# david-knigge/enf-pde

Measured on AMD Instinct MI355X. Metric: query-points/sec (ENF fit+decode) at 64 latents x 64^2 grid, higher is better.
Workload: dtype bf16; 1 GPU; navier_stokes_64x64_z64_b16_per_gpu; decoded_states=1, latents=64, signals_per_gpu=16, inner_steps=3, sampled_points=512, num_hidden=128, num_heads=2, latent_dim=16, num_out=1, invariant=rel_pos_periodic, hparams=config_navier_stokes.yaml:23-96 with 64 latents, parallelism=dp1 (signals sharded, no data-path collective in fit/decode)

## Files before the change

enf-pde_amd/_lib.py:

```python
import ctypes
import os

_HERE = os.path.dirname(os.path.abspath(__file__))
LIB_PATH = os.environ.get("ENF_HIP_LIB") or os.path.join(_HERE, "libenf_hip.so")
TEST_LIB_PATH = os.environ.get("ENF_HIP_TEST_LIB") or os.path.join(_HERE, "libenf_hip_test.so")

ENF_NUM_TENSORS = 46
PREC = {"f32": 0, "fp32": 0, "float32": 0, "bf16": 1, "bfloat16": 1}
INVARIANT_IDS = {"rel_pos_periodic": 0, "latitude_periodic": 1, "polar_periodic": 2, "ponita": 3,
                 "abs_pos": 4, "rel_pos": 5, "norm_rel_pos": 6, "ball": 7, "ball_lat": 8, "ponita_full": 9}

EXPORTS = ["enf_abi_version", "enf_strerror", "enf_invariant_dim", "enf_invariant_pose_dim", "enf_check_desc",
           "enf_packed_weight_bytes", "enf_pack_weights", "enf_workspace_bytes", "enf_forward",
           "enf_backward_latents", "enf_backward_latents_ex", "enf_forward_stages", "enf_lt_layout", "enf_lt_layout_ext", "enf_pack_pair", "enf_pair_forward",
           "enf_pair_backward", "enf_pair_backward_ex", "enf_pair_scratch_bytes", "enf_pair_variant", "enf_pair_partition", "enf_shared_forward_parts", "enf_shared_backward_applies", "enf_backward_weights", "enf_backward_weights_scratch_bytes",
           "enf_backward_all", "enf_backward_all_scratch_bytes", "enf_fit_step", "enf_fit_inputs",
           "enf_mse_value_grad",
           "enf_workspace_bytes_ex", "enf_fit_step_ex", "enf_mse_value_grad_ex", "enf_mse_scratch_bytes", "enf_pair_backward_ex2",
           "enf_pair_backward_scratch_bytes", "enf_backward_all_scratch_bytes_ex", "enf_backward_weights_ex",
           "enf_backward_weights_scratch_bytes_ex",
           "enf_fit_step_w", "enf_mse_value_grad_w", "enf_fit_inputs_w", "enf_fit_inputs_b",
           "enf_fit_step_cw", "enf_mse_value_grad_cw", "enf_fit_inputs_cw",
           "enf_fit_step_e", "enf_eval_loss", "enf_signal_sum",
           "enf_field_grad_workspace_bytes", "enf_field_grad", "enf_query_vjp",
# ... 160 lines not shown
    lib.enf_pair_forward.argtypes = [dp, vp, i64, vp, vp, vp, vp, vp, sz, vp]
    lib.enf_pair_backward.argtypes = [dp, vp, i64, vp, vp, vp, vp, vp, vp, ctypes.POINTER(vp), vp]
    lib.enf_pair_backward_ex.argtypes = [dp, vp, i64, vp, vp, vp, vp, vp, vp, ctypes.POINTER(vp), vp, vp]
    cu = ctypes.c_uint
    lib.enf_workspace_bytes_ex.restype = sz
    lib.enf_workspace_bytes_ex.argtypes = [dp, cu]
    lib.enf_fit_step_ex.argtypes = [dp, vp, i64, vp, vp, vp, vp, vp, ctypes.c_float, vp, vp, vp, vp, vp, sz, cu, vp]
    lib.enf_mse_scratch_bytes.restype = sz
    lib.enf_mse_scratch_bytes.argtypes = [sz, cu]
    lib.enf_mse_value_grad_ex.argtypes = [vp, vp, sz, ctypes.c_float, vp, vp, vp, sz, cu, vp]
    lib.enf_fit_step_w.argtypes = [dp, vp, i64, vp, vp, vp, vp, vp, ctypes.c_float, vp, vp, vp, vp, vp, sz, vp, cu, vp]
    lib.enf_mse_value_grad_w.argtypes = [vp, vp, vp, sz, ctypes.c_int32, ctypes.c_float, vp, vp, vp, sz, cu, vp]
    lib.enf_fit_inputs_w.argtypes = [ctypes.c_int, ctypes.POINTER(EnfFitComponent)] + [ctypes.c_int32] * 7 + [vp] * 9
    lib.enf_fit_inputs_b.argtypes = [ctypes.c_int, ctypes.POINTER(EnfFitComponent)] + [ctypes.c_int32] * 7 + [vp] * 9
    lib.enf_fit_step_cw.argtypes = [dp, vp, i64, vp, vp, vp, vp, vp, ctypes.c_float, vp, vp, vp, vp, vp, sz, vp, cu, vp]
    lib.enf_mse_value_grad_cw.argtypes = [vp, vp, vp, sz, ctypes.c_float, vp, vp, vp, sz, cu, vp]
    lib.enf_fit_inputs_cw.argtypes = [ctypes.c_int, ctypes.POINTER(EnfFitComponent)] + [ctypes.c_int32] * 7 + [vp] * 8 + [ctypes.c_int32, vp]
    lib.enf_fit_step_e.argtypes = [dp, vp, i64, vp, vp, vp, vp, vp, ctypes.c_float, vp, vp, vp, vp, vp, sz, vp, vp, vp, vp, cu, vp]
    lib.enf_eval_loss.argtypes = [dp, vp, i64] + [vp] * 11 + [sz, cu, vp]
    lib.enf_signal_sum.argtypes = [vp, ctypes.c_int32, ctypes.c_int32, ctypes.c_float, vp, vp]
    lib.enf_field_grad_workspace_bytes.restype = sz
    lib.enf_field_grad_workspace_bytes.argtypes = [dp, cu]
    lib.enf_field_grad.argtypes = [dp, vp, i64] + [vp] * 7 + [sz, cu, vp]
    lib.enf_query_vjp.argtypes = [dp, vp, i64] + [vp] * 8 + [sz, cu, vp]
    lib.enf_pair_backward_scratch_bytes.restype = sz
    lib.enf_pair_backward_scratch_bytes.argtypes = [dp, cu]
    lib.enf_pair_backward_ex2.argtypes = [dp, vp, i64, vp, vp, vp, vp, vp, vp, ctypes.POINTER(vp), vp, vp, sz, cu, vp]
    lib.enf_backward_all_scratch_bytes_ex.restype = sz
    lib.enf_backward_all_scratch_bytes_ex.argtypes = [dp, ci, cu]
    lib.enf_backward_weights_scratch_bytes_ex.restype = sz
    lib.enf_backward_weights_scratch_bytes_ex.argtypes = [dp, ci, cu]
    lib.enf_backward_weights_ex.argtypes = [dp, vp, i64, vp, vp, vp, vp, vp, vp, ctypes.POINTER(vp), vp, vp, sz, cu, vp]
    if test_hooks:
        for name in ("enf_debug_gemm", "enf_debug_pack", "enf_test_read_wave_sums"):
            getattr(lib, name).restype = ci
        lib.enf_debug_gemm.argtypes = [vp, vp, vp, ci, ci, ci, vp]
        lib.enf_debug_pack.argtypes = [vp, vp, ci, ci, ci, vp]
        lib.enf_test_read_wave_sums.argtypes = [vp]
    if lib.enf_abi_version() != 2:
        raise EnfError(f"{path}: ABI version mismatch")
    return lib


def check(rc):
    if rc == 0:
        return
    msg = load().enf_strerror(rc).decode()
    if rc == -2:
        raise ValueError(msg)
    if rc == -6:
        raise AssertionError(msg)
    if rc == -3:
        raise NotImplementedError(msg)
    raise EnfError(f"libenf_hip error {rc}: {msg}")


def launch(dev, fn, *args):
    import torch
    idx = dev.index if dev.index is not None else torch.cuda.current_device()
    if idx == torch.cuda.current_device():
        return check(fn(*args))
    with torch.cuda.device(idx):
        return check(fn(*args))


def ptr(t):
    return ctypes.c_void_p(t.data_ptr()) if t is not None else ctypes.c_void_p(0)

# ... 19 lines not shown
```

enf-pde_amd/csrc/enf_device.h:

```cpp
#pragma once
#include <hip/hip_runtime.h>
#include <type_traits>

#define DEV __device__ __forceinline__

typedef float f32x4 __attribute__((ext_vector_type(4)));
typedef __bf16 bf16x8 __attribute__((ext_vector_type(8)));
typedef __bf16 bf16x4 __attribute__((ext_vector_type(4)));
typedef unsigned int u32x4 __attribute__((ext_vector_type(4)));

constexpr int NWAVES = 8;
constexpr int NTHREADS = 64 * NWAVES;

template <bool BF16, int KB>
struct Frags {
  using T = typename std::conditional<BF16, bf16x8, f32x4>::type;
  T f[BF16 ? KB : 2 * KB];
};

typedef float f32x2_cvt __attribute__((ext_vector_type(2)));
typedef __bf16 bf16x2_cvt __attribute__((ext_vector_type(2)));
DEV unsigned bf16_pack2(float a, float b) {
  return __builtin_bit_cast(unsigned, __builtin_convertvector(f32x2_cvt{a, b}, bf16x2_cvt));
}
// ... 325 lines not shown
      const unsigned a = (unsigned)(uintptr_t)(lds_ptr_t)(const_cast<char*>(slot) + (lane << 4));
      f32x4 af[C::MTS];
      if constexpr (INIT == INIT_ZERO) {
        G::run_flip_zero(af, F.f, a);
      } else {
#pragma unroll
        for (int mt = 0; mt < C::MTS; ++mt) af[mt] = flip_init(sp * C::MTS + mt);
        G::run_flip(af, F.f, a);
      }
#pragma unroll
      for (int mt = 0; mt < C::MTS; ++mt) flip(sp * C::MTS + mt, af[mt]);
    } else {
      if constexpr (TRANS) gemm_stage<BF16, KBIN, C::MTS, INIT>(&acc[sp * C::MTS], F, slot, lane, bias + 16 * sp * C::MTS);
#pragma unroll
      for (int mt = 0; mt < C::MTS; ++mt) {
        f32x4 af = flip_init(sp * C::MTS + mt);
        gemm_tile_flip<BF16, KBIN>(af, F, slot, mt, lane);
        flip(sp * C::MTS + mt, af);
      }
    }
    if constexpr (LA) stage_close_la<NEXT_BYTES, NW>(P, ring, next, lane);
    else stage_close(P);
  }
}


template <int BYTES, int NW = NWAVES>
DEV void first_stage(Pipe& P, char* ring, unsigned panel, int wave, int lane) {
  P.cur = 0;
  P.wave = __builtin_amdgcn_readfirstlane(wave);
  P.early = false;
  stage_issue_p<BYTES, NW>(P, panel, ring, lane);
  if (!P.early) { stage_wait(); __syncthreads(); }
}

template <int NT> DEV void tiles_sum_sq(const f32x4 (&X)[NT], float& s, float& q) {
  f32x2 s2 = {0.f, 0.f}, q2 = {0.f, 0.f};
#pragma unroll
  for (int t = 0; t < NT; ++t) {
    const f32x2 a = lo2(X[t]), b = hi2(X[t]);
    s2 += a; q2 = __builtin_elementwise_fma(a, a, q2);
    s2 += b; q2 = __builtin_elementwise_fma(b, b, q2);
  }
  s = s2[0] + s2[1]; q = q2[0] + q2[1];
}
template <int NT, typename GetB> DEV void tiles_sum_dot(const f32x4 (&A)[NT], GetB get, float& s, float& d) {
  f32x2 s2 = {0.f, 0.f}, d2 = {0.f, 0.f};
#pragma unroll
  for (int t = 0; t < NT; ++t) {
    const f32x4 bt = get(t);
    s2 += lo2(A[t]); d2 = __builtin_elementwise_fma(lo2(A[t]), lo2(bt), d2);
    s2 += hi2(A[t]); d2 = __builtin_elementwise_fma(hi2(A[t]), hi2(bt), d2);
  }
  s = s2[0] + s2[1]; d = d2[0] + d2[1];
}

template <int NT, typename GetA, typename GetB> DEV float tiles_dot(GetA geta, GetB getb) {
  f32x2 d2 = {0.f, 0.f};
#pragma unroll
  for (int t = 0; t < NT; ++t) {
    const f32x4 at = geta(t), bt = getb(t);
    d2 = __builtin_elementwise_fma(lo2(at), lo2(bt), d2);
    d2 = __builtin_elementwise_fma(hi2(at), hi2(bt), d2);
  }
  return d2[0] + d2[1];
}
// ... 110 lines not shown
```

enf-pde_amd/csrc/enf_pair_fwd.hip:

```cpp
#include <hip/hip_runtime.h>
#include "enf_launch.h"
#include "enf_device.h"
#include "enf_pair_common.h"

struct PairFwdArgs {
  const float* x; long long x_bstride;
  const float* lt; const char* blob; EnfLayout L;
  float* ybar; float* lse;
  const char* wz; const float* wzb; const char* wzu;
  float inv_d;
  int xcd_remap;
  unsigned* masks; int mask_mode, mask_B;
  int B, N, Z, dx, inv, use_window, qg;
  int zsplit;
  int sk_len;
  int ybar_half;
  float* ysplit;
  float* spart;
  int parts, bcast;
};

#ifdef ENF_STAMPS
__device__ unsigned long long enf_stamps[8 * 4 * 24];
#define STAMP(k)                                                                                              \
  do {                                                                                                        \
    if (blockIdx.x == 7 && blockIdx.y == 0 && lane == 0 && it < 4)                                            \
      enf_stamps[(wave * 4 + it) * 24 + (k)] = __builtin_amdgcn_s_memtime();                                  \
  } while (0)
extern "C" int enf_debug_read_stamps(unsigned long long* dst) {
  return hipMemcpyFromSymbol(dst, HIP_SYMBOL(enf_stamps), sizeof(enf_stamps)) == hipSuccess ? 0 : -1;
}
#else
#define STAMP(k) do {} while (0)
#endif

#define K2_BIAS(ACC, PTR)                                                              \
  do {                                                                                 \
    _Pragma("unroll") for (int t_ = 0; t_ < NT; ++t_) ACC[t_] = rowvec(PTR, t_, quad);   \
  } while (0)
#define K2_MASK_MODE (MASKS && !FFN ? A.mask_mode : 0)
#ifndef ENF_ZFOLD_WAVES
#define ENF_ZFOLD_WAVES 8
#endif

template <bool ZFOLD> struct PairWaves { static constexpr int NW = ZFOLD && ENF_ZFOLD_WAVES == 4 ? 4 : NWAVES; };

template <int D, int H, bool BF16, int NW, bool FFN = false> struct PairSmem {
  static constexpr int RING = 0;
  static constexpr int EW = FFN ? 4 * D : 2 * D;
  static constexpr int CONSTS = RING + 2 * STAGE_MAX;
  static constexpr int N_CONST = 4 * D + 2 * H * D + 2 * EW;
  static constexpr int ZVEC = CONSTS + 4 * N_CONST;
  static constexpr int XCH = ZVEC + 4 * NW * 2 * H * D;
  static constexpr int TOTAL = XCH + 4 * NW * H * 3 * 16;
  static constexpr int YBYTES = H * (D / 16) * 4 * 64 * 4;
  static_assert(4 * YBYTES <= 2 * STAGE_MAX, "combine buffer must fit in the ring");
};

template <int D, int H, bool BF16, bool ZFOLD, bool MASKS, int INV = -1, bool FFN = false>
__global__ __launch_bounds__(64 * PairWaves<ZFOLD>::NW, 2) void enf_pair_fwd_kernel(PairFwdArgs A) {
  const int inv_id = INV >= 0 ? INV : A.inv;
  const int dx_ = INV >= 0 ? 2 : A.dx;
  using Cfg = PairCfg<D, BF16>;
  constexpr int NW = PairWaves<ZFOLD>::NW, NTH = 64 * NW;
  using SM = PairSmem<D, H, BF16, NW, FFN>;
  constexpr int KB = Cfg::KB, NT = Cfg::NT;
  constexpr int ST_DD = Cfg::DD::STAGE, ST_GB = Cfg::GB::STAGE, PANEL_GB = Cfg::GB::BYTES, PANEL_DD = Cfg::DD::BYTES;
  extern __shared__ __attribute__((aligned(16))) char smem[];
  char* ring = smem + SM::RING;
  float* cst = reinterpret_cast<float*>(smem + SM::CONSTS);
  float* c_bq1 = cst, *c_bv1 = cst + D, *c_bf = cst + 2 * D, *c_bm = cst + 3 * D, *c_bgb = cst + 4 * D;
  float* c_acq = c_bgb + 2 * H * D, *c_acv = c_acq + SM::EW;
  const int tid = threadIdx.x, lane = tid & 63, wave = tid >> 6, col = lane & 15, quad = lane >> 4;
  float* zv = reinterpret_cast<float*>(smem + SM::ZVEC) + wave * 2 * H * D;
  float* xch = reinterpret_cast<float*>(smem + SM::XCH);
  const int QG = A.qg, ZS = NW / QG;
  const int qgi = wave % QG, zs = wave / QG;
  int bx = blockIdx.x, by = blockIdx.y;
  if (ZFOLD && A.xcd_remap) {
    const int id = blockIdx.y * gridDim.x + blockIdx.x, xcd = id & 7, slot = id >> 3;
    by = xcd + 8 * (slot / (int)gridDim.x);
    bx = slot % (int)gridDim.x;
  }
  const bool split = ZFOLD && A.zsplit > 1;
  const bool shared = !ZFOLD && A.spart != nullptr;
  const int tiles_n = (A.N + 16 * QG - 1) / (16 * QG);
  int f0 = split ? (int)blockIdx.x * A.sk_len : 0;
  const int f1 = split ? min(f0 + A.sk_len, tiles_n * A.B * A.Z) : 0;
  const char* blob = A.blob;
  auto G = [&](size_t off) { return reinterpret_cast<const float*>(blob + off); };

  for (int i = tid; i < D; i += NTH) { c_bq1[i] = G(A.L.bq1)[i]; c_bv1[i] = G(A.L.bv1)[i]; c_bf[i] = G(A.L.bf)[i]; c_bm[i] = G(A.L.bm)[i]; }
  for (int i = tid; i < 2 * H * D; i += NTH) c_bgb[i] = G(A.L.bgb)[i];
  for (int i = tid; i < SM::EW; i += NTH) { c_acq[i] = G(A.L.acq)[i]; c_acv[i] = G(A.L.acv)[i]; }

  const unsigned pQ1 = (unsigned)A.L.aq1, pV1 = (unsigned)A.L.av1, pF = (unsigned)A.L.af, pGB = (unsigned)A.L.agb, pM = (unsigned)A.L.am;
  const unsigned pFirst = FFN ? pF : pQ1;
  Pipe P;
  P.rs = make_blob_rsrc(blob, (unsigned)A.L.total);
  float sm_m[H], sm_l[H], sm_c[H];
  f32x4 Y[H][NT];
  int b, n0;
 for (;;) {
  int z_lo = 0, seg_iters = 0, part = 0;
  if (split) {
    const int tf = f0 / A.Z;
    z_lo = f0 - tf * A.Z;
    seg_iters = min(A.Z - z_lo, f1 - f0);
    part = (int)blockIdx.x - (tf * A.Z) / A.sk_len;
    by = tf / tiles_n;
    bx = tf - by * tiles_n;
    f0 += seg_iters;
  }
  b = shared ? 0 : by;
  n0 = (bx * QG + qgi) * 16;
  const int n = min(n0 + col, A.N - 1);
  const QueryPt q = load_query(A.x + (size_t)b * A.x_bstride + (size_t)n * dx_, dx_, inv_id);
  if constexpr (ZFOLD) P.rs2 = make_blob_rsrc(A.wz + (size_t)b * A.Z * H * PANEL_DD, (unsigned)(A.Z * H * PANEL_DD));
  else P.rs2 = P.rs;
  first_stage<ST_DD, NW>(P, ring, pFirst, wave, lane);
  auto zgemm = [&](f32x4 (&acc_)[NT], const Frags<BF16, KB>& F_, unsigned panel_, unsigned next_, bool active_, const float* bias_) {
    panel_gemm<KB, NT, BF16, ST_DD, NW, INIT_ACC>(acc_, F_, P, ring, panel_, next_, active_, lane, bias_);
  };

#pragma unroll
  for (int h = 0; h < H; ++h) {
    sm_m[h] = -INFINITY; sm_l[h] = 0.f; sm_c[h] = 0.f;
#pragma unroll
    for (int t = 0; t < NT; ++t) Y[h][t] = f32x4{0.f, 0.f, 0.f, 0.f};
  }

  const int ltstride = enf_lt_stride(H, D);
  const int zpart = shared ? (A.Z + A.parts - 1) / A.parts : A.Z;
  const int z_first = shared ? by * zpart : 0, z_end = shared ? min(z_first + zpart, A.Z) : A.Z;
  const int iters = split ? seg_iters : ZFOLD ? A.Z : (zpart + ZS - 1) / ZS;
  for (int it = 0; it < iters; ++it) {
    const int z = ZFOLD ? z_lo + it : z_first + it * ZS + zs;
    const bool active = z < z_end;
    const float* ltrow = A.lt + ((size_t)b * A.Z + (active ? z : A.Z - 1)) * ltstride;
    STAMP(0);
    if constexpr (ZFOLD) {
      const float* czrow = A.wzb + ((size_t)b * A.Z + z) * (H * D);
#pragma unroll
      for (int i = lane * 4; i < H * D; i += 256) {
        if constexpr (!BF16) *reinterpret_cast<f32x4*>(zv + i) = *reinterpret_cast<const f32x4*>(ltrow + i);
        *reinterpret_cast<f32x4*>(zv + H * D + i) = *reinterpret_cast<const f32x4*>(czrow + i);
      }
      if constexpr (BF16) {
        if (lane < KB * 4 * H)
          *reinterpret_cast<f32x4*>(zv + lane * 4) =
              *reinterpret_cast<const f32x4*>(A.wzu + ((size_t)b * A.Z + z) * enf_wzu_bytes(H, D) + lane * 16);
      }
    } else {
#pragma unroll
      for (int i = lane * 4; i < 2 * H * D; i += 256)
        *reinterpret_cast<f32x4*>(zv + i) = *reinterpret_cast<const f32x4*>(ltrow + i);
    }
    const f32x4 pz = *reinterpret_cast<const f32x4*>(ltrow + enf_lt_off_pose(H, D));
    const float wcoef = ltrow[enf_lt_off_wcoef(H, D)];
    __builtin_amdgcn_fence(__ATOMIC_RELEASE, "wavefront");
    __builtin_amdgcn_fence(__ATOMIC_ACQUIRE, "wavefront");

    float inv[4], win;
    const bool has_ph = INV < 0 && D == 64 && enf_inv_has_phase(inv_id);
    pair_invariant<BF16>(inv_id, dx_, q, pz, wcoef, A.use_window, inv, win, ltrow + enf_lt_off_ext(H, D));

    float logit[H];
    Frags<BF16, KB> F;
    {
      f32x4 acc[NT];
      if constexpr (FFN) {
        ffn_pre<D>(acc, inv, c_acq, c_bq1, col, quad);
        gelu_tiles<NT>(acc);
      } else {
        rff_embed<D, BF16>(acc, inv, c_acq, lane, quad, has_ph ? ltrow + enf_lt_off_phq(H, D) : nullptr);
        make_frags<BF16, KB>(F, acc);
        K2_BIAS(acc, c_bq1);
        STAMP(1);
        if constexpr (ZFOLD) zgemm(acc, F, pQ1, pV1, active, c_bq1);
        else panel_gemm<KB, NT, BF16, ST_DD, NW, INIT_ACC>(acc, F, P, ring, pQ1, pV1, active, lane, c_bq1);
      }
      STAMP(2);
      const bool mread = FFN || K2_MASK_MODE == 2;
      if (K2_MASK_MODE) {
        const size_t mrow = relu_mask_index(b % A.mask_B, A.Z, active ? z : A.Z - 1, (A.N + 15) / 16, n0 / 16, 0, lane);
        if (K2_MASK_MODE == 1 && active && n0 < A.N) A.masks[mrow] = relu_mask_of<NT>(acc);
        if (mread) relu_apply_mask<NT>(acc, n0 < A.N ? A.masks[mrow] : 0u);
      }
      if constexpr (ZFOLD && BF16) {
        static_assert(H <= 4, "logit rows live in one quad");
        make_frags<BF16, KB>(F, acc);
        if (!mread) relu_frags<BF16, KB>(F);
        f32x4 lg = {0.f, 0.f, 0.f, 0.f};
#pragma unroll
        for (int blk = 0; blk < KB; ++blk) {
          bf16x8 ua = __builtin_bit_cast(bf16x8, f32x4{0.f, 0.f, 0.f, 0.f});
          if (col < H) ua = *reinterpret_cast<const bf16x8*>(zv + ((blk * 4 + quad) * H + col) * 4);
          lg = __builtin_amdgcn_mfma_f32_16x16x32_bf16(ua, F.f[blk], lg, 0, 0, 0);
        }
#pragma unroll
        for (int h = 0; h < H; ++h) logit[h] = __shfl(lg[h], col, 64) + ltrow[enf_lt_off_c(H, D) + h] + win;
      } else
#pragma unroll
      for (int h = 0; h < H; ++h) {
        float s = 0.f;
#pragma unroll
        for (int t = 0; t < NT; ++t) {
          const f32x4 u = rowvec(zv + h * D, t, quad);
#pragma unroll
          for (int i = 0; i < 4; ++i) s = fmaf(mread ? acc[t][i] : relu_f(acc[t][i]), u[i], s);
        }
        logit[h] = xquad_sum(s) + ltrow[enf_lt_off_c(H, D) + h] + win;
      }
    }
    STAMP(3);
    {
      f32x4 acc[NT];
      if constexpr (FFN) {
        ffn_pre<D>(acc, inv, c_acv, c_bv1, col, quad);
        gelu_tiles<NT>(acc);
      } else {
        rff_embed<D, BF16>(acc, inv, c_acv, lane, quad, has_ph ? ltrow + enf_lt_off_phv(H, D) : nullptr);
        make_frags<BF16, KB>(F, acc);
        K2_BIAS(acc, c_bv1);
        STAMP(4);
        if constexpr (ZFOLD) zgemm(acc, F, pV1, pF, active, c_bv1);
        else panel_gemm<KB, NT, BF16, ST_DD, NW, INIT_ACC>(acc, F, P, ring, pV1, pF, active, lane, c_bv1);
      }
      STAMP(5);
      const bool mread = FFN || K2_MASK_MODE == 2;
      if (K2_MASK_MODE) {
        const size_t mrow = relu_mask_index(b % A.mask_B, A.Z, active ? z : A.Z - 1, (A.N + 15) / 16, n0 / 16, 1, lane);
        if (K2_MASK_MODE == 1 && active && n0 < A.N) A.masks[mrow] = relu_mask_of<NT>(acc);
        if (mread) relu_apply_mask<NT>(acc, n0 < A.N ? A.masks[mrow] : 0u);
      }
      make_frags<BF16, KB>(F, acc);
      if (!mread) relu_frags<BF16, KB>(F);
      K2_BIAS(acc, c_bf);
      STAMP(6);
      if constexpr (ZFOLD) {
        const unsigned wz0 = STAGE_RS2 | (unsigned)(z * H * PANEL_DD);
        const unsigned after = H > 1 ? wz0 + PANEL_DD : (it + 1 < iters ? pQ1 : NO_STAGE);
        (void)after;
        zgemm(acc, F, pF, wz0, active, c_bf);
      }
      else panel_gemm<KB, NT, BF16, ST_GB, NW, INIT_ACC>(acc, F, P, ring, pF, pGB, active, lane, c_bf);
      STAMP(7);
      gelu_tiles<NT>(acc);
      float mu, rstd;
      ln_stats<NT>(acc, mu, rstd, A.inv_d);
      ln_apply<NT>(acc, mu, rstd);
      make_frags<BF16, KB>(F, acc);
      STAMP(8);
    }
#pragma unroll
    for (int h = 0; h < H; ++h) {
      f32x4 v[NT];
      if constexpr (ZFOLD) {
        const unsigned wzh = STAGE_RS2 | (unsigned)((z * H + h) * PANEL_DD);
        K2_BIAS(v, zv + H * D + h * D);
        STAMP(10 + 4 * h);
        const bool more = it + 1 < iters;
        const unsigned nx1 = h + 1 < H ? wzh + PANEL_DD : (more ? pFirst : NO_STAGE);
        zgemm(v, F, wzh, nx1, active, zv + H * D + h * D);
      } else {
        f32x4 dummy[1];
        gb_panel<D, BF16, ST_DD, false, NW>(v, dummy, F, P, ring, pGB + h * PANEL_GB, pM, active, c_bgb + 2 * h * D,
                                        zv + H * D + h * D, lane, quad);
        STAMP(9 + 4 * h);
        Frags<BF16, KB> FV;
        make_frags<BF16, KB>(FV, v);
        K2_BIAS(v, c_bm);
        STAMP(10 + 4 * h);
        if (h + 1 < H) panel_gemm<KB, NT, BF16, ST_GB, NW, INIT_ACC>(v, FV, P, ring, pM, pGB + (h + 1) * PANEL_GB, active, lane, c_bm);
        else panel_gemm<KB, NT, BF16, ST_DD, NW, INIT_ACC>(v, FV, P, ring, pM, it + 1 < iters ? pFirst : NO_STAGE, active, lane, c_bm);
      }
      STAMP(11 + 4 * h);
      gelu_tiles<NT>(v);
      float mu, rstd;
      ln_stats<NT>(v, mu, rstd, A.inv_d);
      if (active) {
        if (it == 0) sm_m[h] = logit[h];
        const bool far = logit[h] - sm_m[h] > 40.0f;
        if (__any(far)) {
          const float alpha = far ? __expf(sm_m[h] - logit[h]) : 1.0f;
          sm_l[h] *= alpha; sm_c[h] *= alpha;
          if (far) sm_m[h] = logit[h];
#pragma unroll
          for (int t = 0; t < NT; ++t)
#pragma unroll
            for (int i = 0; i < 4; ++i) Y[h][t][i] *= alpha;
        }
        const float pe = __expf(logit[h] - sm_m[h]);
        const float w = pe * rstd;
        sm_l[h] += pe;
        sm_c[h] = fmaf(w, mu, sm_c[h]);
#pragma unroll
        for (int t = 0; t < NT; ++t)
#pragma unroll
          for (int i = 0; i < 4; ++i) Y[h][t][i] = fmaf(w, v[t][i], Y[h][t][i]);
      }
      STAMP(12 + 4 * h);
    }
  }

  pipe_finish(P);
  if constexpr (ZFOLD) {
    if (split) {
// ... 125 lines not shown
  ybar[(size_t)row * HD + c] = (y - C) / L;
  if (c % D == 0) lse[(size_t)row * H + h] = ms + __logf(L);
}

__global__ __launch_bounds__(256) void enf_shared_merge_kernel(const float* __restrict__ part, int P, int N, int H, int D, int bcast,
                                                              float* __restrict__ ybar, float* __restrict__ lse) {
  const int HD = H * D, Q = HD / 4;
  const long long e = (long long)blockIdx.x * blockDim.x + threadIdx.x;
  if (e >= (long long)N * Q) return;
  const int row = (int)(e / Q), c = (int)(e % Q) * 4, h = c / D;
  const float* st = part + (size_t)P * N * HD;
  float ms = -INFINITY;
  for (int r = 0; r < P; ++r) ms = fmaxf(ms, st[((size_t)r * N + row) * (H * 3) + h * 3]);
  float L = 0.f, C = 0.f;
  f32x4 y = {0.f, 0.f, 0.f, 0.f};
  for (int r = 0; r < P; ++r) {
    const float* q = st + ((size_t)r * N + row) * (H * 3) + h * 3;
    const float aw = q[0] == -INFINITY ? 0.f : __expf(q[0] - ms);
    const f32x4 yr = *reinterpret_cast<const f32x4*>(part + ((size_t)r * N + row) * HD + c);
    L = fmaf(aw, q[1], L);
    C = fmaf(aw, q[2], C);
#pragma unroll
    for (int i = 0; i < 4; ++i) y[i] = fmaf(aw, yr[i], y[i]);
  }
#pragma unroll
  for (int i = 0; i < 4; ++i) y[i] = (y[i] - C) / L;
  const float ls = ms + __logf(L);
  for (int b = blockIdx.y; b < bcast; b += gridDim.y) {
    *reinterpret_cast<f32x4*>(ybar + ((size_t)b * N + row) * HD + c) = y;
    if (c % D == 0) lse[((size_t)b * N + row) * H + h] = ls;
  }
}

template <int D, int H, bool BF16, bool ZFOLD, bool MASKS = false, int INV = -1, bool FFN = false>
static int launch_pair_fwd(const PairFwdArgs& A, hipStream_t st) {
  if constexpr (!MASKS && !FFN) {
    if (A.mask_mode) return launch_pair_fwd<D, H, BF16, ZFOLD, true>(A, st);
  }
  constexpr int NW = PairWaves<ZFOLD>::NW;
  using SM = PairSmem<D, H, BF16, NW, FFN>;
  auto kern = enf_pair_fwd_kernel<D, H, BF16, ZFOLD, MASKS, INV, FFN>;
  static EnfAttrBits attr_done{0};
  if (!enf_lds_attr(reinterpret_cast<const void*>(kern), SM::TOTAL, attr_done)) return ENF_ELAUNCH;
  dim3 grid((A.N + 16 * A.qg - 1) / (16 * A.qg), A.B);
  if (ZFOLD && A.zsplit > 1) grid = dim3((unsigned)(((long long)grid.x * A.B * A.Z + A.sk_len - 1) / A.sk_len));
  const bool shared = !ZFOLD && A.spart != nullptr;
  if (shared) grid.y = (unsigned)A.parts;
  hipLaunchKernelGGL(kern, grid, dim3(64 * NW), SM::TOTAL, st, A);
  if (shared) {
    const long long tot = (long long)A.N * (H * D / 4);
    hipLaunchKernelGGL(enf_shared_merge_kernel, dim3((unsigned)((tot + 255) / 256), (unsigned)(A.bcast < 4 ? A.bcast : 4)), dim3(256), 0, st,
                       (const float*)A.spart, A.parts, A.N, H, D, A.bcast, A.ybar, A.lse);
  }
  if (ZFOLD && A.zsplit > 1) {
    const long long BN = (long long)A.B * A.N, tot = BN * H * D;
    hipLaunchKernelGGL(enf_zsplit_merge_kernel, dim3((unsigned)((tot + 255) / 256)), dim3(256), 0, st, (const float*)A.ysplit, A.zsplit, BN, H, D,
                       A.N, A.Z, A.sk_len, A.ybar, A.lse);
  }
  return hipGetLastError() == hipSuccess ? 0 : ENF_ELAUNCH;
}

int enf_launch_pair_fwd(const EnfDims& m, const EnfLayout& L, const char* blob, const float* x, long long x_bstride,
                        const float* lt, float* ybar, float* lse, char* wz, float* wzb, char* wzu, float* ysplit,
                        int run_fold, int run_pair, hipStream_t st, float* spart) {
  PairFwdArgs A;
  A.x = x; A.x_bstride = x_bstride; A.lt = lt; A.blob = blob; A.L = L; A.ybar = ybar; A.lse = lse; A.wz = wz; A.wzb = wzb; A.wzu = wzu; A.inv_d = 1.0f / (float)m.Dt;
  A.B = m.B; A.N = m.N; A.Z = m.Z; A.dx = m.dx; A.inv = m.inv; A.use_window = m.use_window;
  A.masks = m.masks; A.mask_mode = (run_pair & 1) && !m.ffn ? m.mask_mode : 0; A.mask_B = m.mask_B;
  static_assert(NWAVES == 8, "enf_latent_splits (enf_layout.h) splits 8 waves");
  A.qg = NWAVES / enf_latent_splits(m.Z);
  const bool zfold = wz && wzb && wzu && (size_t)m.Z * m.H * enf_panel_bytes(m.D, m.D, m.bf16) < 0x7fffffffu;
  const EnfStreamK sk = enf_zfold_streamk(m);
  A.zsplit = zfold && ysplit && sk.parts > 1 ? sk.parts : 1;
  A.sk_len = A.zsplit > 1 ? sk.len : 0;
// ... 52 lines not shown
```

enf-pde_amd/fitting/ode_models/ponita_ode_g.py:

```python
import math
import os

import torch
import torch.nn.functional as Fnn

from ... import _lib


_ptr, _stream = _lib.ptr, _lib.stream


SPLIT_K = 4096


def _xt_dot(X, G):
    P = X.shape[0]
    n = P // SPLIT_K
    if n < 2:
        return X.t() @ G
    out = torch.bmm(X[:n * SPLIT_K].view(n, SPLIT_K, -1).transpose(1, 2), G[:n * SPLIT_K].view(n, SPLIT_K, -1)).sum(0)
    if n * SPLIT_K < P:
        out = out + X[n * SPLIT_K:].t() @ G[n * SPLIT_K:]
    return out

# ... 244 lines not shown
                    _ptr(out), _stream(inv.device))
        ctx.save_for_backward(inv, aw, u, w, Wi)
        ctx.c = (cr, cs)
        return out

    @staticmethod
    def backward(ctx, g):
        lib = _lib.load()
        inv, aw, u, w, Wi = ctx.saved_tensors
        B, Z, _, I = inv.shape
        D = u.shape[-1]
        g = g.contiguous()
        dinv, daw, du, dw = torch.empty_like(inv), torch.empty_like(aw), torch.empty_like(u), torch.empty_like(w)
        part = torch.empty((B * ((Z + 63) // 64), I), device=inv.device, dtype=torch.float32)
        _lib.launch(inv.device, lib.enf_ode_vec_readout_backward, B, Z, I, D, _ptr(inv), _ptr(aw), _ptr(u), _ptr(w), ctx.c[0], ctx.c[1],
                    _ptr(Wi), _ptr(g), _ptr(dinv), _ptr(daw), _ptr(du), _ptr(dw), _ptr(part), _stream(inv.device))
        return dinv, daw, du, dw, part.sum(0), None, None


FUSED_READOUT = os.environ.get("ENF_ODE_UNFUSED_READOUT", "0") != "1"


def _trunc_normal(gen, shape, std, device):
    t = torch.empty(shape, dtype=torch.float32)
    torch.nn.init.trunc_normal_(t, 0.0, 1.0, -2.0, 2.0, generator=gen)
    return (t * (std / 0.87962566103423978)).to(device)


def _lecun(gen, n_in, n_out, device, bias=True):
    p = {"kernel": _trunc_normal(gen, (n_in, n_out), math.sqrt(1.0 / n_in), device)}
    if bias:
        p["bias"] = torch.zeros(n_out, device=device)
    return p


def _flatten_tree(tree):
    def leaves(t):
        out = []
        for k in sorted(t):
            out += leaves(t[k]) if isinstance(t[k], dict) else [t[k]]
        return out

    def build(lv):
        it = iter(lv)

        def rec(t):
            return {k: (rec(t[k]) if isinstance(t[k], dict) else next(it)) for k in sorted(t)}
        return rec(tree)
    return leaves(tree), build


class PonitaGen:
    def __init__(self, num_hidden, num_layers, scalar_num_out, vec_num_out, invariant, basis_dim, degree, widening_factor,
                 global_pool, kernel_size="global"):
        assert kernel_size == "global" or kernel_size > 0, "kernel_size must be 'global' or a positive number."
        self.num_hidden, self.num_layers, self.scalar_num_out, self.vec_num_out = num_hidden, num_layers, scalar_num_out, vec_num_out
        self.invariant, self.basis_dim, self.degree, self.widening_factor = invariant, basis_dim, degree, widening_factor
        self.global_pool, self.kernel_size = global_pool, kernel_size
        self.poly = PolynomialFeatures(degree)

    def init(self, key, latent_dim, device="cuda"):
        gen = torch.Generator().manual_seed(int(key))
        inv, H, J = self.invariant, self.num_hidden, self.basis_dim
        P = {"kernel_basis": {"layers_1": _lecun(gen, self.poly.num_features(inv.dim), H, device),
                              "layers_3": _lecun(gen, H, J, device)},
             "a_stem": _lecun(gen, latent_dim, H, device, bias=False)}
# ... 52 lines not shown
                vec_out = (readout(P["readout_vec_rel"]["kernel"]) * (p[:, :, None, :zp] - p[:, None, :, :zp])).mean(-2)
            if inv.num_z_ori_dims > 0:
                if fused and p.shape[-1] - zp in (2, 3):
                    vec_out = vec_out + fused_readout(P["readout_vec_ori"]["kernel"], p[..., zp:], p[..., zp:], 0.0, 1.0)
                else:
                    vec_out = vec_out + (readout(P["readout_vec_ori"]["kernel"]) * p[:, None, :, zp:]).mean(-2)
        if self.global_pool:
            scalar_out = scalar_out.mean(1)
            vec_out = vec_out.mean(1) if vec_out is not None else None
        return scalar_out, vec_out


class PonitaODEGen:

    def __init__(self, num_hidden, num_layers, scalar_num_out, vec_num_out, invariant, basis_dim, degree, widening_factor,
                 global_pool, kernel_size="global"):
        self.invariant = invariant
        self.scalar_num_out = scalar_num_out
        n_sc = scalar_num_out + 1 if invariant.num_z_ori_dims > 0 else scalar_num_out
        self.ponita = PonitaGen(num_hidden, num_layers, n_sc, vec_num_out, invariant, basis_dim, degree, widening_factor,
                                global_pool, kernel_size)

    def init(self, key, latents, device=None):
        p, a, _ = latents
        return {"params": {"ponita": self.ponita.init(key, a.shape[-1], device or a.device)}}

    def load_params(self, tree, device="cuda"):
        conv = lambda t: {k: conv(v) for k, v in t.items()} if isinstance(t, dict) else \
            torch.as_tensor(t, dtype=torch.float32).to(device).contiguous()
        return conv(tree)

    def graphed(self, params, latents):
        static_in = tuple(None if v is None else v.detach().clone() for v in latents)
        with torch.no_grad():
            side = torch.cuda.Stream()
            side.wait_stream(torch.cuda.current_stream())
            with torch.cuda.stream(side):
                for _ in range(2):
                    self.apply(params, static_in)
            torch.cuda.current_stream().wait_stream(side)
            graph = torch.cuda.CUDAGraph()
            with torch.cuda.graph(graph):
                static_out = self.apply(params, static_in)

        def f(z):
            for dst, src in zip(static_in, z):
                if dst is not None:
                    dst.copy_(src)
            graph.replay()
            return tuple(None if v is None else v.clone() for v in static_out)
        f.graph = graph
        return f

    def graphed_train(self, params, latents, n):
        leaves, build = _flatten_tree(params)
        p0, a0, w0 = latents

        def fn(p, a, *lv):
            dp, da, _ = self.apply(build(lv), (p, a, w0))
            return dp, da

        fresh = lambda t: t.detach().clone().requires_grad_(True)
        samples = tuple((fresh(p0), fresh(a0), *leaves) for _ in range(n))
        graphed = torch.cuda.make_graphed_callables((fn,) * n, samples, allow_unused_input=True)
        graphed = graphed if isinstance(graphed, tuple) else (graphed,)

        def wrap(g):
            def f(z):
                p, a, w = z
                dp, da = g(p if p.requires_grad else p.detach().requires_grad_(True),
                           a if a.requires_grad else a.detach().requires_grad_(True), *leaves)
                return dp, da, (torch.zeros_like(w) if w is not None else None)
            return f
        return [wrap(g) for g in graphed]

    def apply(self, params, latents):
        p, a, window = latents
        scalar, vec = self.ponita(params["params"]["ponita"], (p, a - 1, window))
        if self.invariant.num_z_ori_dims > 0:
            da, dp = scalar[..., :-1], torch.cat([vec, scalar[..., -1:]], -1)
        else:
            da, dp = scalar, vec
        return dp, da, (torch.zeros_like(window) if window is not None else None)
```

Baseline: 30.89 million query-points/s.

## Keep selected pair-forward weight panels resident in LDS instead of streaming per latent

Adds a compile-time greedy selector that chooses which of the Q1, V1, F and M weight panels fit in the leftover LDS of the pair forward kernel. The chosen panels are loaded once per block and their GEMMs read straight from LDS, so the per-latent ring refill for them is skipped. The streaming prefetch chain is rewired to skip resident panels. The cost is a larger LDS footprint per block, which may reduce occupancy, plus an up-front load. A test hook forces the old streamed path, and a gc.collect runs before graph capture.

After: 31.22 million query-points/s (median of 6 runs). 1.1% higher.

```diff
diff --git a/enf-pde_amd/_lib.py b/enf-pde_amd/_lib.py
--- a/enf-pde_amd/_lib.py
+++ b/enf-pde_amd/_lib.py
@@ -216,8 +216,9 @@
     lib.enf_backward_weights_scratch_bytes_ex.argtypes = [dp, ci, cu]
     lib.enf_backward_weights_ex.argtypes = [dp, vp, i64, vp, vp, vp, vp, vp, vp, ctypes.POINTER(vp), vp, vp, sz, cu, vp]
     if test_hooks:
-        for name in ("enf_debug_gemm", "enf_debug_pack", "enf_test_read_wave_sums"):
+        for name in ("enf_debug_gemm", "enf_debug_pack", "enf_test_read_wave_sums", "enf_test_pair_fwd_streamed"):
             getattr(lib, name).restype = ci
+        lib.enf_test_pair_fwd_streamed.argtypes = [ci]
         lib.enf_debug_gemm.argtypes = [vp, vp, vp, ci, ci, ci, vp]
         lib.enf_debug_pack.argtypes = [vp, vp, ci, ci, ci, vp]
         lib.enf_test_read_wave_sums.argtypes = [vp]
diff --git a/enf-pde_amd/csrc/enf_device.h b/enf-pde_amd/csrc/enf_device.h
--- a/enf-pde_amd/csrc/enf_device.h
+++ b/enf-pde_amd/csrc/enf_device.h
@@ -381,6 +381,24 @@
   P.early = false;
   stage_issue_p<BYTES, NW>(P, panel, ring, lane);
   if (!P.early) { stage_wait(); __syncthreads(); }
+}
+
+template <int BYTES, int NW = NWAVES>
+DEV void resident_load(__amdgpu_buffer_rsrc_t rs, unsigned src_off, char* dst, int wave, int lane) {
+  constexpr int CH = BYTES < STAGE_MAX ? BYTES : STAGE_MAX;
+  static_assert(BYTES % CH == 0, "resident panel: whole staging rounds");
+#pragma unroll
+  for (int o = 0; o < BYTES; o += CH) stage_issue<CH, NW>(rs, src_off + o, dst + o, wave, lane);
+}
+template <int KBIN, int MTOUT, bool BF16, int INIT = INIT_ACC>
+DEV void resident_gemm(f32x4 (&acc)[MTOUT], const Frags<BF16, KBIN>& F, const char* panel, bool active, int lane,
+                       const float* bias = nullptr) {
+  using C = PanelCfg<KBIN, MTOUT, BF16>;
+  static_assert(INIT == INIT_ACC, "resident_gemm: the caller initialises the accumulators");
+  asm volatile("" : "+v"(lane));
+#pragma unroll
+  for (int sp = 0; sp < C::SPP; ++sp)
+    if (active) gemm_stage<BF16, KBIN, C::MTS, INIT>(&acc[sp * C::MTS], F, panel + sp * C::STAGE, lane, bias + 16 * sp * C::MTS);
 }
 
 template <int NT> DEV void tiles_sum_sq(const f32x4 (&X)[NT], float& s, float& q) {
diff --git a/enf-pde_amd/csrc/enf_pair_fwd.hip b/enf-pde_amd/csrc/enf_pair_fwd.hip
--- a/enf-pde_amd/csrc/enf_pair_fwd.hip
+++ b/enf-pde_amd/csrc/enf_pair_fwd.hip
@@ -45,25 +45,55 @@
 
 template <bool ZFOLD> struct PairWaves { static constexpr int NW = ZFOLD && ENF_ZFOLD_WAVES == 4 ? 4 : NWAVES; };
 
-template <int D, int H, bool BF16, int NW, bool FFN = false> struct PairSmem {
+enum { RP_Q1 = 0, RP_V1 = 1, RP_F = 2, RP_M = 3, RP_COUNT = 4 };
+constexpr int LDS_PER_CU = 160 * 1024;
+constexpr unsigned pair_resident_set(const int (&saved)[RP_COUNT], const int (&bytes)[RP_COUNT], int room) {
+  unsigned set = 0;
+  for (int n = 0; n < RP_COUNT; ++n) {
+    int best = -1;
+    for (int i = 0; i < RP_COUNT; ++i) {
+      if ((set >> i & 1u) || saved[i] <= 0 || bytes[i] > room) continue;
+      if (best < 0 || saved[i] > saved[best] || (saved[i] == saved[best] && bytes[i] < bytes[best])) best = i;
+    }
+    if (best < 0) break;
+    set |= 1u << best;
+    room -= bytes[best];
+  }
+  return set;
+}
+constexpr int pair_resident_end(unsigned set, const int (&bytes)[RP_COUNT], int p, int base) {
+  for (int i = 0; i < p; ++i) base += (set >> i & 1u) ? bytes[i] : 0;
+  return base;
+}
+
+template <int D, int H, bool BF16, int NW, bool FFN = false, bool ZFOLD = false, bool RES = true> struct PairSmem {
   static constexpr int RING = 0;
   static constexpr int EW = FFN ? 4 * D : 2 * D;
   static constexpr int CONSTS = RING + 2 * STAGE_MAX;
   static constexpr int N_CONST = 4 * D + 2 * H * D + 2 * EW;
   static constexpr int ZVEC = CONSTS + 4 * N_CONST;
   static constexpr int XCH = ZVEC + 4 * NW * 2 * H * D;
-  static constexpr int TOTAL = XCH + 4 * NW * H * 3 * 16;
+  static constexpr int RESIDENT = XCH + 4 * NW * H * 3 * 16;
   static constexpr int YBYTES = H * (D / 16) * 4 * 64 * 4;
   static_assert(4 * YBYTES <= 2 * STAGE_MAX, "combine buffer must fit in the ring");
+  static constexpr int PANEL = PanelCfg<D / 32, D / 16, BF16>::BYTES, SPP = PanelCfg<D / 32, D / 16, BF16>::SPP;
+  static constexpr int ONE = SPP == 1 ? 1 : 0;
+  static constexpr int SAVED[RP_COUNT] = {FFN ? 0 : ONE, FFN ? 0 : ONE, ONE, ZFOLD ? 0 : H * ONE};
+  static constexpr int BYTES[RP_COUNT] = {PANEL, PANEL, PANEL, PANEL};
+  static constexpr unsigned SET = RES && RESIDENT <= LDS_PER_CU ? pair_resident_set(SAVED, BYTES, LDS_PER_CU - RESIDENT) : 0u;
+  static constexpr bool has(int p) { return SET >> p & 1u; }
+  static constexpr int off(int p) { return pair_resident_end(SET, BYTES, p, RESIDENT); }
+  static constexpr int TOTAL = pair_resident_end(SET, BYTES, RP_COUNT, RESIDENT);
+  static_assert(TOTAL <= LDS_PER_CU, "K2's LDS (ring + constants + resident panels) exceeds one CU's");
 };
 
-template <int D, int H, bool BF16, bool ZFOLD, bool MASKS, int INV = -1, bool FFN = false>
+template <int D, int H, bool BF16, bool ZFOLD, bool MASKS, int INV = -1, bool FFN = false, bool RES = true>
 __global__ __launch_bounds__(64 * PairWaves<ZFOLD>::NW, 2) void enf_pair_fwd_kernel(PairFwdArgs A) {
   const int inv_id = INV >= 0 ? INV : A.inv;
   const int dx_ = INV >= 0 ? 2 : A.dx;
   using Cfg = PairCfg<D, BF16>;
   constexpr int NW = PairWaves<ZFOLD>::NW, NTH = 64 * NW;
-  using SM = PairSmem<D, H, BF16, NW, FFN>;
+  using SM = PairSmem<D, H, BF16, NW, FFN, ZFOLD, RES && NW == NWAVES>;
   constexpr int KB = Cfg::KB, NT = Cfg::NT;
   constexpr int ST_DD = Cfg::DD::STAGE, ST_GB = Cfg::GB::STAGE, PANEL_GB = Cfg::GB::BYTES, PANEL_DD = Cfg::DD::BYTES;
   extern __shared__ __attribute__((aligned(16))) char smem[];
@@ -95,9 +125,21 @@
   for (int i = tid; i < SM::EW; i += NTH) { c_acq[i] = G(A.L.acq)[i]; c_acv[i] = G(A.L.acv)[i]; }
 
   const unsigned pQ1 = (unsigned)A.L.aq1, pV1 = (unsigned)A.L.av1, pF = (unsigned)A.L.af, pGB = (unsigned)A.L.agb, pM = (unsigned)A.L.am;
-  const unsigned pFirst = FFN ? pF : pQ1;
   Pipe P;
   P.rs = make_blob_rsrc(blob, (unsigned)A.L.total);
+  constexpr bool rQ1 = SM::has(RP_Q1), rV1 = SM::has(RP_V1), rF = SM::has(RP_F), rM = SM::has(RP_M);
+  constexpr int oQ1 = SM::off(RP_Q1), oV1 = SM::off(RP_V1), oF = SM::off(RP_F), oM = SM::off(RP_M);
+  {
+    const int wv = __builtin_amdgcn_readfirstlane(wave);
+    if constexpr (rQ1) resident_load<PANEL_DD, NW>(P.rs, pQ1, smem + oQ1, wv, lane);
+    if constexpr (rV1) resident_load<PANEL_DD, NW>(P.rs, pV1, smem + oV1, wv, lane);
+    if constexpr (rF) resident_load<PANEL_DD, NW>(P.rs, pF, smem + oF, wv, lane);
+    if constexpr (rM) resident_load<PANEL_DD, NW>(P.rs, pM, smem + oM, wv, lane);
+  }
+  constexpr bool sQ1 = !FFN && !rQ1, sV1 = !FFN && !rV1, sF = !rF;
+  auto first_from = [&](int pos, unsigned at3) { return sQ1 && pos <= 0 ? pQ1 : sV1 && pos <= 1 ? pV1 : sF && pos <= 2 ? pF : at3; };
+  constexpr int ST_3 = ZFOLD ? ST_DD : ST_GB;
+  constexpr int ST_FROM0 = sQ1 || sV1 || sF ? ST_DD : ST_3, ST_FROM1 = sV1 || sF ? ST_DD : ST_3, ST_FROM2 = sF ? ST_DD : ST_3;
   float sm_m[H], sm_l[H], sm_c[H];
   f32x4 Y[H][NT];
   int b, n0;
@@ -118,9 +160,13 @@
   const QueryPt q = load_query(A.x + (size_t)b * A.x_bstride + (size_t)n * dx_, dx_, inv_id);
   if constexpr (ZFOLD) P.rs2 = make_blob_rsrc(A.wz + (size_t)b * A.Z * H * PANEL_DD, (unsigned)(A.Z * H * PANEL_DD));
   else P.rs2 = P.rs;
-  first_stage<ST_DD, NW>(P, ring, pFirst, wave, lane);
+  auto wzp = [&](int zz, int h_) { return STAGE_RS2 | (unsigned)((zz * H + h_) * PANEL_DD); };
+  first_stage<ST_FROM0, NW>(P, ring, first_from(0, ZFOLD ? wzp(z_lo, 0) : pGB), wave, lane);
   auto zgemm = [&](f32x4 (&acc_)[NT], const Frags<BF16, KB>& F_, unsigned panel_, unsigned next_, bool active_, const float* bias_) {
     panel_gemm<KB, NT, BF16, ST_DD, NW, INIT_ACC>(acc_, F_, P, ring, panel_, next_, active_, lane, bias_);
+  };
+  auto rgemm = [&](f32x4 (&acc_)[NT], const Frags<BF16, KB>& F_, int off_, bool active_, const float* bias_) {
+    resident_gemm<KB, NT, BF16, INIT_ACC>(acc_, F_, smem + off_, active_, lane, bias_);
   };
 
 #pragma unroll
@@ -137,6 +183,8 @@
   for (int it = 0; it < iters; ++it) {
     const int z = ZFOLD ? z_lo + it : z_first + it * ZS + zs;
     const bool active = z < z_end;
+    const unsigned at3 = ZFOLD ? wzp(z, 0) : pGB;
+    const unsigned wrap = it + 1 < iters ? first_from(0, ZFOLD ? wzp(z + 1, 0) : pGB) : NO_STAGE;
     const float* ltrow = A.lt + ((size_t)b * A.Z + (active ? z : A.Z - 1)) * ltstride;
     STAMP(0);
     if constexpr (ZFOLD) {
@@ -177,8 +225,8 @@
         make_frags<BF16, KB>(F, acc);
         K2_BIAS(acc, c_bq1);
         STAMP(1);
-        if constexpr (ZFOLD) zgemm(acc, F, pQ1, pV1, active, c_bq1);
-        else panel_gemm<KB, NT, BF16, ST_DD, NW, INIT_ACC>(acc, F, P, ring, pQ1, pV1, active, lane, c_bq1);
+        if constexpr (rQ1) rgemm(acc, F, oQ1, active, c_bq1);
+        else panel_gemm<KB, NT, BF16, ST_FROM1, NW, INIT_ACC>(acc, F, P, ring, pQ1, first_from(1, at3), active, lane, c_bq1);
       }
       STAMP(2);
       const bool mread = FFN || K2_MASK_MODE == 2;
@@ -224,8 +272,8 @@
         make_frags<BF16, KB>(F, acc);
         K2_BIAS(acc, c_bv1);
         STAMP(4);
-        if constexpr (ZFOLD) zgemm(acc, F, pV1, pF, active, c_bv1);
-        else panel_gemm<KB, NT, BF16, ST_DD, NW, INIT_ACC>(acc, F, P, ring, pV1, pF, active, lane, c_bv1);
+        if constexpr (rV1) rgemm(acc, F, oV1, active, c_bv1);
+        else panel_gemm<KB, NT, BF16, ST_FROM2, NW, INIT_ACC>(acc, F, P, ring, pV1, first_from(2, at3), active, lane, c_bv1);
       }
       STAMP(5);
       const bool mread = FFN || K2_MASK_MODE == 2;
@@ -238,13 +286,8 @@
       if (!mread) relu_frags<BF16, KB>(F);
       K2_BIAS(acc, c_bf);
       STAMP(6);
-      if constexpr (ZFOLD) {
-        const unsigned wz0 = STAGE_RS2 | (unsigned)(z * H * PANEL_DD);
-        const unsigned after = H > 1 ? wz0 + PANEL_DD : (it + 1 < iters ? pQ1 : NO_STAGE);
-        (void)after;
-        zgemm(acc, F, pF, wz0, active, c_bf);
-      }
-      else panel_gemm<KB, NT, BF16, ST_GB, NW, INIT_ACC>(acc, F, P, ring, pF, pGB, active, lane, c_bf);
+      if constexpr (rF) rgemm(acc, F, oF, active, c_bf);
+      else panel_gemm<KB, NT, BF16, ST_3, NW, INIT_ACC>(acc, F, P, ring, pF, at3, active, lane, c_bf);
       STAMP(7);
       gelu_tiles<NT>(acc);
       float mu, rstd;
@@ -260,20 +303,21 @@
         const unsigned wzh = STAGE_RS2 | (unsigned)((z * H + h) * PANEL_DD);
         K2_BIAS(v, zv + H * D + h * D);
         STAMP(10 + 4 * h);
-        const bool more = it + 1 < iters;
-        const unsigned nx1 = h + 1 < H ? wzh + PANEL_DD : (more ? pFirst : NO_STAGE);
-        zgemm(v, F, wzh, nx1, active, zv + H * D + h * D);
+        zgemm(v, F, wzh, h + 1 < H ? wzh + PANEL_DD : wrap, active, zv + H * D + h * D);
       } else {
         f32x4 dummy[1];
-        gb_panel<D, BF16, ST_DD, false, NW>(v, dummy, F, P, ring, pGB + h * PANEL_GB, pM, active, c_bgb + 2 * h * D,
-                                        zv + H * D + h * D, lane, quad);
+        const float* gbias = c_bgb + 2 * h * D, *v0 = zv + H * D + h * D;
+        if constexpr (!rM) gb_panel<D, BF16, ST_DD, false, NW>(v, dummy, F, P, ring, pGB + h * PANEL_GB, pM, active, gbias, v0, lane, quad);
+        else if (h + 1 < H) gb_panel<D, BF16, ST_GB, false, NW>(v, dummy, F, P, ring, pGB + h * PANEL_GB, pGB + (h + 1) * PANEL_GB, active, gbias, v0, lane, quad);
+        else gb_panel<D, BF16, ST_FROM0, false, NW>(v, dummy, F, P, ring, pGB + h * PANEL_GB, wrap, active, gbias, v0, lane, quad);
         STAMP(9 + 4 * h);
         Frags<BF16, KB> FV;
         make_frags<BF16, KB>(FV, v);
         K2_BIAS(v, c_bm);
         STAMP(10 + 4 * h);
-        if (h + 1 < H) panel_gemm<KB, NT, BF16, ST_GB, NW, INIT_ACC>(v, FV, P, ring, pM, pGB + (h + 1) * PANEL_GB, active, lane, c_bm);
-        else panel_gemm<KB, NT, BF16, ST_DD, NW, INIT_ACC>(v, FV, P, ring, pM, it + 1 < iters ? pFirst : NO_STAGE, active, lane, c_bm);
+        if constexpr (rM) rgemm(v, FV, oM, active, c_bm);
+        else if (h + 1 < H) panel_gemm<KB, NT, BF16, ST_GB, NW, INIT_ACC>(v, FV, P, ring, pM, pGB + (h + 1) * PANEL_GB, active, lane, c_bm);
+        else panel_gemm<KB, NT, BF16, ST_FROM0, NW, INIT_ACC>(v, FV, P, ring, pM, wrap, active, lane, c_bm);
       }
       STAMP(11 + 4 * h);
       gelu_tiles<NT>(v);
@@ -465,14 +509,24 @@
   }
 }
 
-template <int D, int H, bool BF16, bool ZFOLD, bool MASKS = false, int INV = -1, bool FFN = false>
+#ifdef ENF_TEST_HOOKS
+static int g_test_streamed = 0;
+extern "C" int enf_test_pair_fwd_streamed(int on) { const int was = g_test_streamed; g_test_streamed = on != 0; return was; }
+#endif
+
+template <int D, int H, bool BF16, bool ZFOLD, bool MASKS = false, int INV = -1, bool FFN = false, bool RES = true>
 static int launch_pair_fwd(const PairFwdArgs& A, hipStream_t st) {
   if constexpr (!MASKS && !FFN) {
     if (A.mask_mode) return launch_pair_fwd<D, H, BF16, ZFOLD, true>(A, st);
   }
+#ifdef ENF_TEST_HOOKS
+  if constexpr (RES) {
+    if (g_test_streamed) return launch_pair_fwd<D, H, BF16, ZFOLD, MASKS, INV, FFN, false>(A, st);
+  }
+#endif
   constexpr int NW = PairWaves<ZFOLD>::NW;
-  using SM = PairSmem<D, H, BF16, NW, FFN>;
-  auto kern = enf_pair_fwd_kernel<D, H, BF16, ZFOLD, MASKS, INV, FFN>;
+  using SM = PairSmem<D, H, BF16, NW, FFN, ZFOLD, RES && NW == NWAVES>;
+  auto kern = enf_pair_fwd_kernel<D, H, BF16, ZFOLD, MASKS, INV, FFN, RES>;
   static EnfAttrBits attr_done{0};
   if (!enf_lds_attr(reinterpret_cast<const void*>(kern), SM::TOTAL, attr_done)) return ENF_ELAUNCH;
   dim3 grid((A.N + 16 * A.qg - 1) / (16 * A.qg), A.B);
diff --git a/enf-pde_amd/fitting/ode_models/ponita_ode_g.py b/enf-pde_amd/fitting/ode_models/ponita_ode_g.py
--- a/enf-pde_amd/fitting/ode_models/ponita_ode_g.py
+++ b/enf-pde_amd/fitting/ode_models/ponita_ode_g.py
@@ -300,6 +300,11 @@
     if bias:
         p["bias"] = torch.zeros(n_out, device=device)
     return p
+
+
+def _collect_before_capture():
+    import gc
+    gc.collect()
 
 
 def _flatten_tree(tree):
@@ -418,6 +423,7 @@
 
     def graphed(self, params, latents):
         static_in = tuple(None if v is None else v.detach().clone() for v in latents)
+        _collect_before_capture()
         with torch.no_grad():
             side = torch.cuda.Stream()
             side.wait_stream(torch.cuda.current_stream())
@@ -448,6 +454,7 @@
 
         fresh = lambda t: t.detach().clone().requires_grad_(True)
         samples = tuple((fresh(p0), fresh(a0), *leaves) for _ in range(n))
+        _collect_before_capture()
         graphed = torch.cuda.make_graphed_callables((fn,) * n, samples, allow_unused_input=True)
         graphed = graphed if isinstance(graphed, tuple) else (graphed,)
 
```
